# hilo-mpc/hilo-mpc

Measured on AMD Instinct MI355X. Metric: MPC steps/sec (batched instances, whole node) at fixed (nx,nu,N), higher is better.
Workload: dtype f64

## Files before the change

### hilo_mpc_amd/_lib.py

```python
import ctypes as C
import os

HERE = os.path.dirname(os.path.abspath(__file__))
LIB_PATH = os.environ.get('HILO_LIB_PATH') or os.path.join(HERE, 'libhilo_hip.so')

c_double_p = C.c_void_p
c_i64 = C.c_int64


class HiloError(RuntimeError):
    code = 0


class NotPositiveDefinite(HiloError, ValueError):
    code = -5


class KfDesc(C.Structure):
    _fields_ = [('model_id', C.c_int32), ('kind', C.c_int32), ('continuous', C.c_int32), ('erk_order', C.c_int32),
                ('n_sub', C.c_int32), ('lti_nx', C.c_int32), ('lti_nu', C.c_int32), ('lti_ny', C.c_int32),
                ('dt', C.c_double), ('alpha', C.c_double), ('beta', C.c_double), ('kappa', C.c_double),
                ('user_source', C.c_char_p), ('n_user_gp', C.c_int32), ('user_gp', C.c_void_p * 4)]


# ... 45 lines not shown
               [('user_source', C.c_char_p)] + \
               [(n, C.c_int32) for n in ('user_nx', 'user_nu', 'user_np', 'user_ny', 'user_discrete', 'collocation_degree')] + \
               [('coll_A', C.c_void_p), ('coll_D', C.c_void_p), ('n_con', C.c_int32), ('reserved6', C.c_int32), ('con_lb', C.c_void_p),
                ('con_ub', C.c_void_p)]


_lib = None


def _declare(lib):
    vp, i32, i64, dbl = C.c_void_p, C.c_int, C.c_int64, C.c_double
    P = C.POINTER
    sig = {
        'hilo_abi_version': (C.c_int, []),
        'hilo_last_error': (C.c_char_p, []),
        'hilo_device_count': (C.c_int, [P(C.c_int)]),
        'hilo_model_dims': (C.c_int, [i32, P(C.c_int), P(C.c_int), P(C.c_int), P(C.c_int), P(C.c_int)]),
        'hilo_malloc': (C.c_int, [P(vp), C.c_uint64, i32]),
        'hilo_free': (C.c_int, [vp]),
        'hilo_memcpy_h2d': (C.c_int, [vp, vp, C.c_uint64, vp]),
        'hilo_memcpy_d2h': (C.c_int, [vp, vp, C.c_uint64, vp]),
        'hilo_stream_sync': (C.c_int, [vp]),
        'hilo_kf_create': (C.c_int, [P(KfDesc), i32, P(vp)]),
        'hilo_kf_destroy': (None, [vp]),
        'hilo_kf_dims': (C.c_int, [vp, P(C.c_int), P(C.c_int), P(C.c_int), P(C.c_int), P(C.c_int)]),
        'hilo_kf_predict': (C.c_int, [vp, i64, vp, vp, i64, vp, i64, vp, vp]),
        'hilo_kf_update': (C.c_int, [vp, i64, vp, vp, vp, i64, vp, i64, vp, vp, vp]),
        'hilo_kf_step': (C.c_int, [vp, i64, vp, vp, vp, i64, vp, i64, vp, i64, vp, vp, vp]),
        'hilo_pf_function': (C.c_int, [vp, i64, i32, vp, vp, vp, i64, vp, vp, vp, i64, vp, vp, vp, vp]),
        'hilo_model_rollout': (C.c_int, [vp, P(SimOpts), i64, i32, vp, vp, i64, i64, vp, vp, vp, vp]),
        'hilo_model_rollout_resume': (C.c_int, [vp, P(SimOpts), i64, i32, vp, vp, i64, i64, vp, vp, vp, vp, vp]),
        'hilo_model_rollout_dae': (C.c_int, [vp, P(SimOpts), i64, i32, vp, vp, vp, i64, i64, vp, vp, vp, vp, vp]),
        'hilo_model_linearize': (C.c_int, [vp, i64, vp, vp, i64, vp, vp, vp, vp]),
        'hilo_lqr_gain': (C.c_int, [i32, i32, i64, vp, i64, vp, i64, vp, i64, vp, i64, vp, i64, P(LqrOpts), vp, vp, vp, vp]),
        'hilo_lqr_call': (C.c_int, [vp, P(LqrOpts), i64, vp, vp, vp, vp, i64, vp, vp, vp, vp, vp, vp, vp, vp]),
        'hilo_lqr_apply': (C.c_int, [i32, i32, i64, vp, i64, vp, vp, vp, vp, vp]),
        'hilo_pf_stats': (C.c_int, [vp, i64, i32, vp, vp, vp, vp, vp, vp, vp, vp, vp]),
        'hilo_pf_resample': (C.c_int, [vp, i64, i32, vp, vp, vp, vp, vp, vp, vp, vp]),
        'hilo_nmpc_create': (C.c_int, [P(NmpcDesc), i32, P(vp)]),
        'hilo_nmpc_destroy': (None, [vp]),
        'hilo_nmpc_dims': (C.c_int, [vp, P(C.c_int), P(C.c_int), P(C.c_int), P(C.c_int), P(C.c_int)]),
        'hilo_nmpc_reset_warm_start': (C.c_int, [vp]),
        'hilo_nmpc_set_fix_x0': (C.c_int, [vp, i32]),
        'hilo_nmpc_set_x0_box': (C.c_int, [vp, vp, vp]),
        'hilo_nmpc_set_gather': (C.c_int, [vp, vp, i32]),
        'hilo_nmpc_set_plant_out': (C.c_int, [vp, vp]),
        'hilo_nmpc_set_var_bounds': (C.c_int, [vp, vp, vp]),
        'hilo_kf_steps': (C.c_int, [vp, i64, i32, vp, vp, vp, i64, i64, vp, i64, vp, i64, vp, i32, vp, vp]),
        'hilo_kf_steps_split': (C.c_int, [vp, i64, i32, vp, vp, vp, i64, i64, vp, i64, vp, i64, vp, i64, vp, i32, vp, vp]),
        'hilo_nmpc_solve': (C.c_int, [vp, i64, vp, vp, i64, vp, vp, vp, vp, vp, vp, vp, vp, vp, vp]),
        'hilo_nmpc_solve_tv': (C.c_int, [vp, i64, vp, vp, i64, vp, vp, vp, vp, vp, vp, vp, vp, vp, vp]),
        'hilo_nmpc_profile': (C.c_int, [vp, i32, vp]),
        'hilo_nmpc_layout_capacity': (C.c_int, [i32, i32, P(C.c_int), P(C.c_longlong), P(C.c_longlong)]),
        'hilo_nmpc_plant_step': (C.c_int, [vp, i64, vp, vp, vp, i64, vp, vp]),
        'hilo_jit_precompile': (C.c_int, [C.c_char_p] + [i32] * 11),
        'hilo_nmpc_set_aux_outputs': (C.c_int, [vp, vp, vp]),
        'hilo_gp_set_mean_program': (C.c_int, [vp, vp, i32]),
        'hilo_jit_precompile_kf': (C.c_int, [C.c_char_p]),
        'hilo_mhe_create': (C.c_int, [P(MheDesc), i32, P(vp)]),
        'hilo_mhe_destroy': (None, [vp]),
        'hilo_mhe_dims': (C.c_int, [vp] + [P(C.c_int)] * 6),
        'hilo_mhe_reset_warm_start': (C.c_int, [vp]),
        'hilo_mhe_estimate': (C.c_int, [vp, i64, vp, vp, i64, vp, vp, vp, vp, vp, vp, vp, vp, vp, vp, vp]),
        'hilo_qp_create': (C.c_int, [i32, i32, i32, P(vp)]),
        'hilo_qp_destroy': (None, [vp]),
        'hilo_qp_set_options': (C.c_int, [vp, dbl, i32]),
        'hilo_qp_set_stages': (C.c_int, [vp, i32, i32, i32, P(i32)]),
        'hilo_qp_solve': (C.c_int, [vp, i64, vp, i64, vp, i64, vp, i64, vp, vp, i64, vp, vp, i64, vp, vp, vp, vp, vp, vp, vp]),
        'hilo_qp_solve_pinned': (C.c_int, [vp, i64, vp, i64, vp, i64, vp, i64, vp, vp, i64, vp, i32, i64, vp, vp, i64, vp, vp, vp, vp, vp,
                                           vp, vp]),
        'hilo_gp_create': (C.c_int, [i32, i32, i32, vp, vp, vp, i32, vp, i32, dbl, P(vp)]),
        'hilo_gp_destroy': (None, [vp]),
        'hilo_gp_log_marginal_likelihood': (C.c_int, [vp, P(C.c_double)]),
        'hilo_gp_refit': (C.c_int, [vp, vp, i32, dbl]),
        'hilo_gp_lml_gradient': (C.c_int, [vp, i32, vp, vp, vp, vp]),
        'hilo_gp_predict': (C.c_int, [vp, i64, vp, i32, vp, vp, vp]),
        'hilo_gp_kernel_matrix': (C.c_int, [i32, i32, vp, i32, i64, vp, i64, vp, vp, vp]),
        'hilo_gp_mean': (C.c_int, [i32, i32, vp, i32, i64, vp, vp, vp]),
        'hilo_ann_create': (C.c_int, [i32, i32, i32, i32, vp, vp, vp, vp, vp, vp, vp, vp, P(vp)]),
        'hilo_ann_destroy': (None, [vp]),
        'hilo_ann_predict': (C.c_int, [vp, i64, vp, i64, vp, i64, vp]),
    }
    for name, (res, args) in sig.items():
        if not hasattr(lib, name):
            continue
        fn = getattr(lib, name)
        fn.restype = res
        fn.argtypes = args
    return lib


def lib():
    global _lib
    if _lib is None:
        if not os.path.exists(LIB_PATH):
            raise HiloError(f"{LIB_PATH} not found: build it with `python -m hilo_mpc_amd._build` "
                            f"(hipcc --offload-arch=gfx950). hilo_mpc_amd has no CPU fallback.")
        try:
            _lib = _declare(C.CDLL(LIB_PATH))
        except OSError as e:
            raise HiloError(f"cannot load {LIB_PATH}: {e}") from e
    return _lib


COMPILED_ONLY = 1

# ... 12 lines not shown
```

### hilo_mpc_amd/csrc/hilo_nmpc.hip

```cpp
#include <stdlib.h>
#include <string.h>

#include "hilo_nmpc_gen.h"
#include "hilo_nmpc_track.h"

namespace hilo {

template <class M>
__global__ void plant_step_kernel(const OcpConst* __restrict__ pcg, int64_t batch, const double* __restrict__ x,
                                  const double* __restrict__ u, const double* __restrict__ par, int64_t par_stride,
                                  double* __restrict__ xn) {
  const int64_t b = (int64_t)blockIdx.x * blockDim.x + threadIdx.x;
  if (b >= batch) return;
  constexpr int NX = M::NX, NU = M::NU, NP = M::NP;
  double xv[NX], uv[NU > 0 ? NU : 1], pv[NP > 0 ? NP : 1], xo[NX];
#pragma unroll
  for (int i = 0; i < NX; ++i) xv[i] = x[b * NX + i];
#pragma unroll
  for (int i = 0; i < NU; ++i) uv[i] = u[b * NU + i];
#pragma unroll
  for (int i = 0; i < NP; ++i) pv[i] = par[b * par_stride + i];
  if constexpr (model_has_ext<M>::value) {
    const GpExt ext{pcg->ext, nullptr, 1, 0, 0, false};
    model_step<M>(pcg->order, pcg->nsub, xv, uv, pv, pcg->dt, xo, ext);
// ... 579 lines not shown

extern "C" int hilo_nmpc_solve(hilo_nmpc* h, int64_t batch, const double* x0, const double* p, int64_t p_stride,
                               const double* v0, const double* u_old, double* v_opt, double* f_opt, double* lam_g,
                               double* u0, int32_t* status, int32_t* iters, double* kkt, void* stream) {
  return nmpc_solve_impl(h, batch, x0, p, p_stride, nullptr, 0, v0, u_old, v_opt, f_opt, lam_g, u0, status, iters, kkt, stream);
}

extern "C" int hilo_nmpc_solve_tv(hilo_nmpc* h, int64_t batch, const double* x0, const double* stage_data, int64_t sd_stride,
                                  const double* v0, const double* u_old, double* v_opt, double* f_opt, double* lam_g,
                                  double* u0, int32_t* status, int32_t* iters, double* kkt, void* stream) {
  HILO_REQUIRE(h && (h->tv || h->tv_width), "hilo_nmpc_solve_tv: the handle was not created with desc.time_varying");
  HILO_REQUIRE(batch <= 0 || stage_data, "hilo_nmpc_solve_tv: NULL stage data");
  const int64_t need = (int64_t)(h->N + 1) * (h->nx + h->nu + h->np);
  HILO_REQUIRE(sd_stride == 0 || sd_stride >= need, "hilo_nmpc_solve_tv: sd_stride %lld < %lld", (long long)sd_stride,
               (long long)need);
  return nmpc_solve_impl(h, batch, x0, nullptr, 0, stage_data, sd_stride, v0, u_old, v_opt, f_opt, lam_g, u0, status, iters, kkt,
                         stream);
}

extern "C" int hilo_nmpc_profile(hilo_nmpc* h, int enable, long long* cycles_host) {
  HILO_REQUIRE(h, "hilo_nmpc_profile: NULL handle");
  HILO_HIP_CHECK(hipSetDevice(h->device));
  if (cycles_host && h->prof) {
    HILO_HIP_CHECK(hipDeviceSynchronize());
    HILO_HIP_CHECK(hipMemcpy(cycles_host, h->prof, sizeof(long long) * PH_COUNT, hipMemcpyDeviceToHost));
  }
  if (enable && !h->prof) {
    HILO_HIP_CHECK(hipMalloc((void**)&h->prof, sizeof(long long) * PH_COUNT));
    HILO_HIP_CHECK(hipMemset(h->prof, 0, sizeof(long long) * PH_COUNT));
  } else if (!enable && h->prof) {
    HILO_HIP_CHECK(hipFree(h->prof));
    h->prof = nullptr;
  }
  return HILO_OK;
}

extern "C" int hilo_nmpc_plant_step(hilo_nmpc* h, int64_t batch, const double* x, const double* u, const double* p,
                                    int64_t p_stride, double* x_next, void* stream) {
  HILO_REQUIRE(h, "hilo_nmpc_plant_step: NULL handle");
  if (batch <= 0) return HILO_OK;
  HILO_REQUIRE(x && u && x_next && (h->np == 0 || p), "hilo_nmpc_plant_step: NULL argument");
  HILO_HIP_CHECK(hipSetDevice(h->device));
  if (h->jit_policy >= 0) return jit_launch_plant(h->jit.plant, h->dev, batch, x, u, p, p_stride, x_next, (hipStream_t)stream);
  const unsigned grid = (unsigned)((batch + 255) / 256);
  switch (h->model_id) {
#define X(ID, T) case ID: hipLaunchKernelGGL((plant_step_kernel<T>), dim3(grid), dim3(256), 0, (hipStream_t)stream, h->dev, batch, x, u, p, p_stride, x_next); break;
    HILO_NMPC_MODELS(X)
#undef X
  }
  HILO_HIP_CHECK(hipGetLastError());
  return HILO_OK;
}

#ifdef HILO_OCP_DPROF
extern "C" int hilo_debug_dprof(long long* out, int reset) {
  if (out) HILO_HIP_CHECK(hipMemcpyFromSymbol(out, HIP_SYMBOL(hilo::g_dprof), sizeof(long long) * 32));
  if (reset) { long long z[32] = {0}; HILO_HIP_CHECK(hipMemcpyToSymbol(HIP_SYMBOL(hilo::g_dprof), z, sizeof(z))); }
  return HILO_OK;
}
#endif
```

### hilo_mpc_amd/csrc/hilo_ocp.h

```cpp
#pragma once
#include "hilo_colloc.h"
#include "hilo_common.h"
#include "hilo_models.h"

namespace hilo {

constexpr int OCP_MAXNX = 12, OCP_MAXNU = 8, OCP_MAXNZ = OCP_MAXNX + OCP_MAXNU;
constexpr int OCP_FILTER = 16;
constexpr int OCP_MAXNC = 16;
#ifndef HILO_OCP_TPB
#define HILO_OCP_TPB 64
#endif
#ifndef HILO_OCP_MINW
#define HILO_OCP_MINW 1
#endif
#ifdef HILO_OCP_INLINE_PHASES
#define OCP_PHASE __attribute__((always_inline))
#else
#define OCP_PHASE __attribute__((noinline))
#endif
#ifndef HILO_OCP_SEAMS
#define HILO_OCP_SEAMS 3
#endif
constexpr int OCP_SEAMS = HILO_OCP_SEAMS;
#ifndef HILO_OCP_LAYOUT_CAP
#define HILO_OCP_LAYOUT_CAP 1
#endif
constexpr bool OCP_LAYOUT_CAP = HILO_OCP_LAYOUT_CAP != 0;
constexpr int OCP_TPB = HILO_OCP_TPB;
constexpr int OCP_NCOST = 2 * OCP_MAXNZ * OCP_MAXNZ + 4 * OCP_MAXNZ + 64;

struct OcpConst {
  int N, order, nsub, max_iter, acceptable_iter, flags;
  int Nc;
  int tail_off;
  double dt;
  double lbz[OCP_MAXNZ], ubz[OCP_MAXNZ];
  double x0lb[OCP_MAXNX], x0ub[OCP_MAXNX];
  double sz[OCP_MAXNZ];
  double tol, acceptable_tol, mu_init, kappa_eps, kappa_mu, theta_mu, tau_min, bound_push, bound_frac, s_max,
      kappa_sigma, gamma_theta, gamma_phi, delta_ls, s_theta, s_phi, eta_phi, theta_min_fact, theta_max_fact,
      delta_w_min, delta_w_0, delta_w_max, kappa_w_minus, kappa_w_plus, kappa_w_plus_bar;
  const double* ext;
  unsigned x0_free_mask;
  unsigned k0_only_mask;
  int nc, nc_term;
  double dlb[OCP_MAXNC], dub[OCP_MAXNC];
  int n_con_ref, n_tcon_ref;
  short row_ref[OCP_MAXNC], trow_ref[OCP_MAXNC];
  CollData coll;
  unsigned long long pair_mask[4];
  double bound_relax;
  double cost[OCP_NCOST];
};

inline void ocp_default_options(OcpConst& c) {
  c.max_iter = 3000; c.acceptable_iter = 15;
  c.tol = 1e-8; c.acceptable_tol = 1e-6; c.mu_init = 0.1;
  c.kappa_eps = 10.0; c.kappa_mu = 0.2; c.theta_mu = 1.5; c.tau_min = 0.99;
  c.bound_push = 1e-2; c.bound_frac = 1e-2; c.s_max = 100.0; c.kappa_sigma = 1e10;
  c.gamma_theta = 1e-5; c.gamma_phi = 1e-8; c.delta_ls = 1.0; c.s_theta = 1.1; c.s_phi = 2.3; c.eta_phi = 1e-8;
  c.theta_min_fact = 1e-4; c.theta_max_fact = 1e4;
  c.delta_w_min = 1e-20; c.delta_w_0 = 1e-4; c.delta_w_max = 1e40; c.kappa_w_minus = 1.0 / 3; c.kappa_w_plus = 8.0;
  c.kappa_w_plus_bar = 100.0;
  for (auto& w : c.pair_mask) w = ~0ull;
}

struct OpSum { static constexpr bool NAN_VOTE = false; __device__ static double id() { return 0.0; } __device__ static double f(double a, double b) { return a + b; } };
__device__ __forceinline__ double nmax(double a, double b) { return (a != a || a > b) ? a : b; }
struct OpMax { static constexpr bool NAN_VOTE = true; __device__ static double id() { return -INFINITY; } __device__ static double f(double a, double b) { return nmax(a, b); } };
struct OpMin { static constexpr bool NAN_VOTE = false; __device__ static double id() { return INFINITY; } __device__ static double f(double a, double b) { return fmin(a, b); } };
struct OpMax2 { static constexpr bool NAN_VOTE = false; __device__ static double id() { return -INFINITY; } __device__ static double f(double a, double b) { return fmax(a, b); } };

template <int CTRL>
__device__ __forceinline__ double dpp_mov(double v) {
// ... 16 lines not shown
  return (int64_t)(((unsigned long long)hi << 32) | lo);
}
__device__ __forceinline__ double uni(double v) {
  return __hiloint2double(__builtin_amdgcn_readfirstlane(__double2hiint(v)), __builtin_amdgcn_readfirstlane(__double2loint(v)));
}
template <class T>
__device__ __forceinline__ __attribute__((address_space(3))) T* uni(__attribute__((address_space(3))) T* p) {
  return (__attribute__((address_space(3))) T*)(size_t)(unsigned)__builtin_amdgcn_readfirstlane((int)(size_t)p);
}
template <class T>
__device__ __forceinline__ T* uni(T* p) {
  const unsigned long long a = (unsigned long long)p;
  const unsigned lo = (unsigned)__builtin_amdgcn_readfirstlane((int)(unsigned)a);
  const unsigned hi = (unsigned)__builtin_amdgcn_readfirstlane((int)(unsigned)(a >> 32));
  return (T*)(((unsigned long long)hi << 32) | lo);
}
#ifndef HILO_RSQ_NEWTON
#define HILO_RSQ_NEWTON 2
#endif
__device__ __forceinline__ double rsq_fast(double x) {
  double y = __builtin_amdgcn_rsq(x);
  const double hx = 0.5 * x;
  y = y * fma(-hx * y, y, 1.5);
  if (HILO_RSQ_NEWTON >= 2) y = y * fma(-hx * y, y, 1.5);
  return y;
}
typedef double v4d __attribute__((ext_vector_type(4)));
struct FTheta { double f, theta, x; };

__device__ __forceinline__ bool wave_any_nan(double v) { return __builtin_amdgcn_ballot_w64(v != v) != 0ull; }
template <class Op>
__device__ __forceinline__ double wave_reduce(double v) {
  if constexpr (Op::NAN_VOTE) {
    const bool nan = wave_any_nan(v);
    const double r = wave_reduce<OpMax2>(v);
    return nan ? __builtin_nan("") : r;
  }
  v = Op::f(v, dpp_mov<0xB1>(v));
  v = Op::f(v, dpp_mov<0x4E>(v));
  v = Op::f(v, dpp_mov<0x141>(v));
  v = Op::f(v, dpp_mov<0x140>(v));
  return uni(Op::f(Op::f(read_lane(v, 0), read_lane(v, 16)), Op::f(read_lane(v, 32), read_lane(v, 48))));
}

enum { R_SUM = 0, R_MAX = 1, R_MIN = 2, R_MAX2 = 3 };
__device__ __forceinline__ double red_apply(int op, double a, double b) {
  switch (op) {
    case R_SUM: return a + b;
    case R_MAX: return fmax(a, b);
    case R_MIN: return fmin(a, b);
    default: return fmax(a, b);
  }
}
template <int... OPS>
struct WaveReduceN {
  static constexpr int n = sizeof...(OPS);
  template <int CTRL>
  __device__ __forceinline__ static void level(double* v) {
    constexpr int ops[n] = {OPS...};
    double t[n];
#pragma unroll
    for (int j = 0; j < n; ++j) t[j] = dpp_mov<CTRL>(v[j]);
#pragma unroll
    for (int j = 0; j < n; ++j) v[j] = red_apply(ops[j], v[j], t[j]);
  }
  __device__ __forceinline__ static void run(double* v) {
    static_assert(OCP_TPB == 64, "one wave per instance");
    constexpr int ops[n] = {OPS...};
    bool nan[n];
#pragma unroll
    for (int j = 0; j < n; ++j) nan[j] = ops[j] == R_MAX && wave_any_nan(v[j]);
    level<0xB1>(v);
    level<0x4E>(v);
    level<0x141>(v);
    level<0x140>(v);
    double a[n], b[n];
#pragma unroll
    for (int j = 0; j < n; ++j) {
      a[j] = red_apply(ops[j], read_lane(v[j], 0), read_lane(v[j], 16));
      b[j] = red_apply(ops[j], read_lane(v[j], 32), read_lane(v[j], 48));
    }
#pragma unroll
    for (int j = 0; j < n; ++j) {
      const double r = uni(red_apply(ops[j], a[j], b[j]));
      v[j] = nan[j] ? __builtin_nan("") : r;
    }
  }
};

template <class Op>
__device__ __forceinline__ double block_reduce(double v, __attribute__((address_space(3))) double* scratch) {
  v = wave_reduce<Op>(v);
  if constexpr (OCP_TPB == 64) return v;
  const int nw = blockDim.x >> 6;
  if (nw == 1) return v;
  __syncthreads();
  if ((threadIdx.x & 63) == 0) scratch[threadIdx.x >> 6] = v;
  __syncthreads();
  double r = Op::id();
  for (int w = 0; w < nw; ++w) r = Op::f(r, scratch[w]);
  return r;
}

template <class MS, class = void> struct sym_masks {
  static constexpr unsigned long long X = ~0ull, J = ~0ull, H = ~0ull;
};
template <class MS> struct sym_masks<MS, void_tt<decltype(MS::HAS_MASKS)>> {
  static constexpr unsigned long long X = MS::HAS_MASKS ? MS::XMASK : ~0ull, J = MS::HAS_MASKS ? MS::JMASK : ~0ull,
                                      H = MS::HAS_MASKS ? MS::HMASK : ~0ull;
};
template <class PB, class = void> struct pb_plant { static constexpr bool value = false; };
template <class PB> struct pb_plant<PB, void_tt<decltype(PB::PLANT)>> { static constexpr bool value = PB::PLANT; };
template <class PB, class = void> struct pb_symtab { static constexpr bool value = false; };
template <class PB> struct pb_symtab<PB, void_tt<decltype(PB::SYMTAB)>> { static constexpr bool value = PB::SYMTAB; };
template <class PB, class = void> struct pb_nh { static constexpr int value = 0; };
template <class PB> struct pb_nh<PB, void_tt<decltype(PB::NH)>> { static constexpr int value = PB::NH; };
template <class PB, class = void> struct pb_sym { static constexpr bool value = false; };
template <class PB> struct pb_sym<PB, void_tt<decltype(PB::SYM)>> { static constexpr bool value = PB::SYM; };
template <class PB, class = void> struct pb_sym_mhe { static constexpr bool value = false; };
template <class PB> struct pb_sym_mhe<PB, void_tt<decltype(PB::SYM_MHE)>> { static constexpr bool value = PB::SYM_MHE; };
template <class PB, class = void> struct pb_vec_n { static constexpr int value = 0; };
template <class PB> struct pb_vec_n<PB, void_tt<decltype(PB::VEC_N)>> { static constexpr int value = PB::VEC_N; };
template <class PB, class = void> struct pb_fused_con { static constexpr bool value = false; };
template <class PB> struct pb_fused_con<PB, void_tt<decltype(PB::FUSED_CON)>> { static constexpr bool value = PB::FUSED_CON; };
template <class PB, class = void> struct pb_prep { static constexpr int value = 0; };
template <class PB> struct pb_prep<PB, void_tt<decltype(PB::PREP)>> { static constexpr int value = PB::PREP; };
template <class PB, class = void> struct pb_vec_max { static constexpr int value = 3; };
template <class PB> struct pb_vec_max<PB, void_tt<decltype(PB::VEC_MAX)>> { static constexpr int value = PB::VEC_MAX; };
template <class PB, class = void> struct pb_cstage { static constexpr int value = 0; };
template <class PB> struct pb_cstage<PB, void_tt<decltype(PB::CSTAGE)>> { static constexpr int value = PB::CSTAGE; };
template <class PB, class = void> struct pb_xcw { static constexpr int value = 0; };
template <class PB> struct pb_xcw<PB, void_tt<decltype(PB::XCW)>> { static constexpr int value = PB::XCW; };
template <class PB, class = void> struct pb_lam_fix { static constexpr bool value = false; };
template <class PB> struct pb_lam_fix<PB, void_tt<decltype(PB::LAM_FIX)>> { static constexpr bool value = PB::LAM_FIX; };
template <class PB, class = void> struct pb_fused { static constexpr bool value = false; };
template <class PB> struct pb_fused<PB, void_tt<decltype(PB::FUSED)>> { static constexpr bool value = PB::FUSED; };
template <class PB, class = void> struct pb_layout_n { static constexpr int value = 0; };
template <class PB> struct pb_layout_n<PB, void_tt<decltype(PB::LAYOUT_N)>> { static constexpr int value = PB::LAYOUT_N; };

__host__ __device__ constexpr size_t ocp_iter_doubles(int NX, int NU, int NC, int N) {
  const size_t NZ = NX + NU, NDIR = NZ * (NZ + 1) / 2, S = (size_t)(N + 1) * NZ;
  return 9 * S + NX + 5 * (size_t)N * NX + (size_t)N * NX * (NZ + 1) + (size_t)N * NZ * (NZ + 1) + (size_t)(N + 1) * NDIR +
         (size_t)(N + 1) * NX * (NX + 1) + (size_t)N * NU * (NX + 1) + (size_t)N * NX * (NX + 1) + (size_t)N * NC * (14 + NZ) +
         (size_t)N * 4 * NX;
}
__host__ __device__ constexpr size_t ocp_fixed_doubles(int NX, int NU, int NCONST, int NPAR, int NSD, int NEXT, int N, int NPREP = 0) {
  const size_t NZ = NX + NU;
  return NCONST + NZ * NZ + NZ + (N + 1) + 2 * 16 + 16 + NPAR + (size_t)(N + 1) * (NSD > 0 ? NSD : 0) + 1 + NEXT +
         (NZ * (NZ + 1) / 2 + 2) / 2 + NPREP;
}

struct OcpExtra {
  const double* par2;
  int npar1;
// ... 1531 lines not shown
          lsum += ok[u] ? fabs(lv[u]) : 0.0;
        }
      }
    }
    double ncon = 0.0;
    if constexpr (NC > 0) {
      OCP_FOR(e, N * NC) {
        const int m = e % NC;
        double sg = 0.0, q = 0.0;
        if (row_on(pc, e / NC, m)) {
          dmax = nmax(dmax, fabs(-l.cnu[e] - l.cvL[e] + l.cvU[e]));
          pmax = nmax(pmax, fabs(l.cd[e] - l.cs[e]));
          th += fabs(l.cd[e] - l.cs[e]);
          lsum += fabs(l.cnu[e]);
          zsum += fabs(l.cvL[e]) + fabs(l.cvU[e]);
          if (pc.dlb[m] > -INFINITY) {
            const double sl = l.cs[e] - pc.dlb[m], is = rcp_fast(sl), p = sl * l.cvL[e];
            cmax = fmax(cmax, p);
            cmin = fmin(cmin, p);
            sg += l.cvL[e] * is;
            q += is;
          }
          if (pc.dub[m] < INFINITY) {
            const double su = pc.dub[m] - l.cs[e], is = rcp_fast(su), p = su * l.cvU[e];
            cmax = fmax(cmax, p);
            cmin = fmin(cmin, p);
            sg += l.cvU[e] * is;
            q -= is;
          }
        }
        l.csig[e] = sg;
        l.crb[e] = q;
      }
      ncon = (double)N * pc.nc + pc.nc_term;
    }
    KktErr r;
    DTICK(12)
    if constexpr (OCP_TPB == 64) {
      double rv[7] = {th, cmax, cmin, dmax, pmax, lsum, zsum};
      WaveReduceN<R_SUM, R_MAX2, R_MIN, R_MAX, R_MAX, R_SUM, R_SUM>::run(rv);
      r.theta = rv[0]; r.pmax = rv[1]; r.pmin = rv[2]; dmax = rv[3]; pmax = rv[4]; lsum = rv[5]; zsum = rv[6];
    } else {
      r.theta = uni(block_reduce<OpSum>(th, l.red));
      r.pmax = uni(block_reduce<OpMax2>(cmax, l.red));
      r.pmin = uni(block_reduce<OpMin>(cmin, l.red));
      dmax = block_reduce<OpMax>(dmax, l.red);
      pmax = block_reduce<OpMax>(pmax, l.red);
      lsum = block_reduce<OpSum>(lsum, l.red);
      zsum = block_reduce<OpSum>(zsum, l.red);
    }
    const double i_smax = rcp_fast(pc.s_max);
    const double s_d = fmax(pc.s_max, (lsum + zsum) * rcp_fast(N * NX + ncon + nb)) * i_smax;
    const double poison = (lsum + zsum + r.theta) * 0.0;
    r.s_c = uni(fmax(pc.s_max, zsum * rcp_fast(nb)) * i_smax + poison);
    r.i_s_c = uni(rcp_fast(r.s_c));
    r.dual_s = uni(dmax * rcp_fast(s_d));
    r.prim = uni(pmax);
    DTICK(13)
    return r;
  }
  __device__ __forceinline__ static double compl_of(const KktErr& r, double mu) { return fmax(fmax(r.pmax - mu, mu - r.pmin), 0.0); }
  __device__ __forceinline__ static bool switching(const OcpConst& pc, double alpha, double nd, double th0) {
    const double dls = pc.delta_ls;
    const bool plain = alpha > 1e-30 && alpha < 1e30 && nd > 1e-100 && nd < 1e100 && th0 > 1e-100 && th0 < 1e100 && dls > 1e-30 && dls < 1e30;
    if (plain) {
      auto lg2 = [](double x) {
        return (double)__builtin_amdgcn_frexp_exp(x) + (double)__builtin_amdgcn_logf((float)__builtin_amdgcn_frexp_mant(x));
      };
      const double d = lg2(alpha) + pc.s_phi * lg2(nd) - lg2(dls) - pc.s_theta * lg2(th0);
      if (fabs(d) > 1e-4) return d > 0.0;
    }
    return alpha * pow(nd, pc.s_phi) > dls * pow(th0, pc.s_theta);
  }
  __device__ static void finish_rhs(const Lds l, double mu) {
    const OcpConst& pc = *(const OcpConst*)l.pc;
    const int N = pc.N;
    {
      constexpr int U = BIG ? 3 : 2;
      const int SLT = (N + 1) * NZ;
      for (int base = 0; base < SLT; base += OCP_TPB * U) {
        double gr[U], qv[U];
        bool ok[U];
#pragma unroll
        for (int u = 0; u < U; ++u) {
          const int e0 = base + u * OCP_TPB + (int)threadIdx.x;
          ok[u] = e0 < SLT;
          const int e = ok[u] ? e0 : 0, k = e / NZ, i = e - k * NZ;
          gr[u] = l.grad[e];
          qv[u] = k < N ? l.W[(size_t)(k * NZ + i) * WP + NZ] : l.rbN[i < NX ? i : 0];
        }
#pragma unroll
        for (int u = 0; u < U; ++u) {
          const int e = base + u * OCP_TPB + (int)threadIdx.x;
          if (!ok[u]) continue;
          const int k = e / NZ, i = e - k * NZ;
          if (k < N) l.W[(size_t)(k * NZ + i) * WP + NZ] = gr[u] - mu * qv[u];
          else if (i < NX) l.rbN[i] = gr[u] - mu * qv[u];
        }
      }
    }
    if constexpr (NC > 0) {
      OCP_FOR(e, N * NC) l.crb[e] = -mu * l.crb[e];
    }
    __syncthreads();
  }
  __device__ static double count_bounds(const Lds l) {
    const OcpConst& pc = *(const OcpConst*)l.pc;
    const int N = pc.N;
    double nb = 0.0;
// ... 980 lines not shown
      if constexpr (NC > 0) {
        OCP_FOR(e, N * NC) {
          const int m = e % NC;
          double sg = 0.0, r = 0.0;
          if (row_on(pc, e / NC, m)) {
            if (pc.dlb[m] > -INFINITY) { const double is = 1.0 / (l.cs[e] - pc.dlb[m]); sg += mu_r * is * is; r -= mu_r * is; }
            if (pc.dub[m] < INFINITY) { const double is = 1.0 / (pc.dub[m] - l.cs[e]); sg += mu_r * is * is; r += mu_r * is; }
          }
          l.csig[e] = sg;
          l.crb[e] = r;
        }
      }
      __syncthreads();
      riccati(lbase, ws, mu, 1.0, true);
      double a = 1.0, dmax = 0.0;
      if constexpr (NC > 0) {
        OCP_FOR(e, N * NC) {
          const int m = e % NC;
          if (!row_on(pc, e / NC, m)) continue;
          const double d = l.cds[e];
          if (pc.dlb[m] > -INFINITY && d < 0.0) a = fmin(a, -tau * (l.cs[e] - pc.dlb[m]) / d);
          if (pc.dub[m] < INFINITY && d > 0.0) a = fmin(a, tau * (pc.dub[m] - l.cs[e]) / d);
        }
      }
      OCP_FOR(e, SL) {
        const double d = l.D[e], lb = l.lbA[e], ub = l.ubA[e], z = l.Z[e];
        dmax = nmax(dmax, fabs(d));
        if (lb > -INFINITY && d < 0.0) a = fmin(a, -tau * (z - lb) / d);
        if (ub < INFINITY && d > 0.0) a = fmin(a, tau * (ub - z) / d);
      }
      double alpha = block_reduce<OpMin>(a, l.red);
      dmax = block_reduce<OpMax>(dmax, l.red);
      if (dmax <= 1e-9 && th > 1e-6) return 2;
      bool ok = false;
      double tht = 0.0, ft = 0.0;
      while (alpha > 1e-10) {
        OCP_FOR(e, SL) l.Zt[e] = l.Z[e] + alpha * l.D[e];
        if constexpr (NC > 0)
          OCP_FOR(e, N * NC) l.cst[e] = l.cs[e] + alpha * l.cds[e];
        __syncthreads();
        const FTheta trial = eval_values(lbase, ws, l.Zt, l.ct, l.cst);
        ft = trial.f; tht = trial.theta;
        if (isfinite(tht) && tht <= (1.0 - 1e-4 * alpha) * th) { ok = true; break; }
        alpha = uni(alpha * 0.5);
      }
      if (!ok) return th > 1e-6 ? 2 : 1;
      OCP_FOR(e, SL) l.Z[e] = l.Zt[e];
      if constexpr (NC > 0)
        OCP_FOR(e, N * NC) l.cs[e] = l.cst[e];
      __syncthreads();
      th = tht;
      if (th <= 0.9 * th_start && th <= theta_max) {
        const double ph = ft + mu * barrier_logs(l, l.Z, l.cs);
        bool acc = true;
        for (int q = 0; q < nfilt; ++q)
          if (th >= l.filt[2 * q] && ph >= l.filt[2 * q + 1]) { acc = false; break; }
        if (acc) return 0;
      }
      eval_derivs(lbase, ws);
    }
    return 1;
  }
  __device__ OCP_PHASE static void load_instance(lds_double* lds_raw_in, double* ws_in, const OcpConst* pcg_in, int64_t b_in,
                                                 const double* x0_in, const double* par_in, int64_t par_stride_in,
                                                 const double* sdata_in, int64_t sd_stride_in, const double* vb_in, int v_prefix_in,
                                                 const double* par2_in, int npar1_in, const double* lbx_in, const double* ubx_in,
                                                 int64_t bx_stride_in) {
    using S = Ocp<PB>;
    constexpr int NTAIL = NX - NXV - NH;
    using gbl_const = const __attribute__((address_space(1))) OcpConst;
    lds_double* const lds_raw = uni(lds_raw_in);
    double* const wsb = uni(ws_in);
    gbl_const* const pcg = (gbl_const*)uni(pcg_in);
    const int64_t b = uni(b_in), par_stride = uni(par_stride_in), sd_stride = uni(sd_stride_in), bx_stride = uni(bx_stride_in);
    gbl_cdouble *const x0 = (gbl_cdouble*)uni(x0_in), *const par = (gbl_cdouble*)uni(par_in), *const sdata = (gbl_cdouble*)uni(sdata_in),
                *const vb = (gbl_cdouble*)uni(vb_in), *const par2 = (gbl_cdouble*)uni(par2_in), *const lbx = (gbl_cdouble*)uni(lbx_in),
                *const ubx = (gbl_cdouble*)uni(ubx_in);
    const int v_prefix = uni(v_prefix_in), npar1 = uni(npar1_in);
    const int t = threadIdx.x;
    const int N = uni(pcg->N);
    const Lds l = carve(lds_raw, wsb, N);
    constexpr int CT = (S::NCONST + OCP_TPB - 1) / OCP_TPB, PT = (PB::NPAR + OCP_TPB - 1) / OCP_TPB;
    gbl_cdouble* const csrc = reinterpret_cast<gbl_cdouble*>(pcg);
    double cbuf[CT], pbuf[PT > 0 ? PT : 1];
#pragma unroll
    for (int j = 0; j < CT; ++j) {
      const int i = j * OCP_TPB + t;
      cbuf[j] = csrc[i < S::NCONST ? i : 0];
    }
    {
      const int n1 = par2 || npar1 > 0 ? npar1 : PB::NPAR;
      const bool has1 = n1 > 0, has2 = par2 != nullptr && n1 < PB::NPAR;
#pragma unroll
      for (int j = 0; j < PT; ++j) {
        const int i = j * OCP_TPB + t;
        const bool p1 = i < PB::NPAR && i < n1, p2 = i < PB::NPAR && !p1 && has2;
        double v1 = 0.0, v2 = 0.0;
        if (has1) v1 = par[b * par_stride + (p1 ? i : 0)];
        if (has2) v2 = par2[b * (int64_t)(PB::NPAR - n1) + (p2 ? i - n1 : 0)];
        pbuf[j] = p1 ? v1 : (p2 ? v2 : 0.0);
      }
    }
    const int SL = (N + 1) * NZ;
    const int flags_g = uni(pcg->flags), tail_g = uni(pcg->tail_off), Ncv = NH > 0 ? uni(pcg->Nc) : N;
    FreeTest is_free_g;
    is_free_g.pinm = uni((int)(FIX_X0 ? (~pcg->x0_free_mask) & ((1u << NX) - 1u) : 0u));
    is_free_g.N = N;
    is_free_g.Nc = NH > 0 ? Ncv : 0;
    const int toff = tail_g > 0 ? tail_g : (N + 1) * NXV + Ncv * NU;
    struct SlotIn { double raw, lo, up; bool pin, bx; };
// ... 276 lines not shown
    if constexpr (NC > 0) {
      OCP_FOR(e, N * NC) {
        const int m = e % NC;
        double dl = 0.0, du = 0.0;
        if (S::row_on(pc, e / NC, m)) {
          const double d = l.cds[e];
          if (pc.dlb[m] > -INFINITY) {
            const double is = rcp_fast(l.cs[e] - pc.dlb[m]), vl = l.cvL[e];
            dl = mu * is - vl - vl * is * d;
            r_p = fmax(r_p, -d * is);
            r_z = fmax(r_z, -dl * rcp_fast(vl));
          }
          if (pc.dub[m] < INFINITY) {
            const double is = rcp_fast(pc.dub[m] - l.cs[e]), vu = l.cvU[e];
            du = mu * is - vu + vu * is * d;
            r_p = fmax(r_p, d * is);
            r_z = fmax(r_z, -du * rcp_fast(vu));
          }
          dphi += l.crb[e] * d;
        }
        l.cdvL[e] = dl;
        l.cdvU[e] = du;
      }
    }
    DTICK(15)
    if constexpr (OCP_TPB == 64) {
      double rv[3] = {r_p, r_z, dphi};
      WaveReduceN<R_MAX, R_MAX, R_SUM>::run(rv);
      r_p = rv[0]; r_z = rv[1]; dphi = rv[2];
    } else {
      r_p = block_reduce<OpMax>(r_p, l.red);
      r_z = block_reduce<OpMax>(r_z, l.red);
      dphi = block_reduce<OpSum>(dphi, l.red);
    }
    const double a_p = uni(r_p > tau ? tau / r_p : 1.0), a_z = uni(r_z > tau ? tau / r_z : 1.0);
    if (!blog_ok) blog = S::barrier_logs(l, l.Z, l.cs);
    const double phi0 = uni(fval + mu * blog);
    DTICK(16)
    OCP_TICK(PH_STEP)
    double alpha = a_p;
    bool accepted = false, armijo = false;
    double blog_t = 0.0, f_acc = 0.0;
    for (int ls = 0; ls < 60; ++ls) {
      DTICKR
      const double blog_part = S::form_trial_part(l, alpha);
      DTICK(17)
      tprof[PH_NLS] += 1;
      const FTheta trial = S::eval_values(lds_raw, wsb, l.Zt, l.ct, l.cst, l.cdt, blog_part);
      blog_t = trial.x;
      DTICK(18)
      const double ft = trial.f, tht = trial.theta;
      const double pht = uni(ft + mu * blog_t);
      bool ok = isfinite(pht) && isfinite(tht) && tht <= theta_max;
      if (ok) {
        for (int q = 0; q < nfilt; ++q) {
          const double tf = l.filt[2 * q], pf = l.filt[2 * q + 1];
          if (tht >= tf && pht - 10 * 2.220446049250313e-16 * fabs(pf) >= pf) { ok = false; break; }
        }
      }
      bool sw = false;
      if (ok) {
        sw = th0 <= theta_min && dphi < 0.0 && S::switching(pc, alpha, -dphi, th0);
        const double rnd = 10 * 2.220446049250313e-16 * fabs(phi0);
        if (sw) ok = pht - phi0 - rnd <= pc.eta_phi * alpha * dphi;
        else ok = tht <= (1 - pc.gamma_theta) * th0 || pht - phi0 - rnd <= -pc.gamma_phi * th0;
      }
      DTICK(19)
      if (ok) { accepted = true; armijo = sw; f_acc = ft; break; }
      if (ls == 0 && tht >= th0) {
        OCP_FOR(e, N * NX) l.c0[e] = l.c[e];
        if constexpr (NC > 0)
          OCP_FOR(e, N * NC) l.cd0[e] = l.cd[e];
        double a_prev = alpha, th_old = tht;
        bool soc_ok = false, soc_sw = false;
        for (int ps = 0; ps < 4; ++ps) {
          OCP_FOR(e, N * NX) l.c[e] = a_prev * l.c[e] + l.ct[e];
          if constexpr (NC > 0) {
            OCP_FOR(e, N * NC) {
              if (S::row_on(pc, e / NC, e % NC)) l.cd[e] = l.cs[e] + a_prev * (l.cd[e] - l.cs[e]) + (l.cdt[e] - l.cst[e]);
            }
          }
          __syncthreads();
          tprof[PH_NRIC] += 1;
          if (!uni(S::riccati(lds_raw, wsb, mu, delta))) break;
          double a = 1.0;
          OCP_FOR(e, SL) {
            const double d = l.D[e], lb = l.lbA[e], ub = l.ubA[e], z = l.Z[e];
            if (lb > -INFINITY && d < 0.0) a = fmin(a, -tau * (z - lb) / d);
            if (ub < INFINITY && d > 0.0) a = fmin(a, tau * (ub - z) / d);
          }
          if constexpr (NC > 0) {
            OCP_FOR(e, N * NC) {
              const int m = e % NC;
              if (!S::row_on(pc, e / NC, m)) continue;
              const double d = l.cds[e];
              if (pc.dlb[m] > -INFINITY && d < 0.0) a = fmin(a, -tau * (l.cs[e] - pc.dlb[m]) / d);
              if (pc.dub[m] < INFINITY && d > 0.0) a = fmin(a, tau * (pc.dub[m] - l.cs[e]) / d);
            }
          }
          const double a_s = block_reduce<OpMin>(a, l.red);
          const double blog_part2 = S::form_trial_part(l, a_s);
          tprof[PH_NLS] += 1;
          const FTheta t2 = S::eval_values(lds_raw, wsb, l.Zt, l.ct, l.cst, l.cdt, blog_part2);
          blog_t = t2.x;
          const double ths = t2.theta;
          const double phs = uni(t2.f + mu * blog_t);
          bool oks = isfinite(phs) && isfinite(ths) && ths <= theta_max;
          if (oks) {
            for (int q = 0; q < nfilt; ++q) {
              const double tf = l.filt[2 * q], pf = l.filt[2 * q + 1];
              if (ths >= tf && phs - 10 * 2.220446049250313e-16 * fabs(pf) >= pf) { oks = false; break; }
            }
          }
          if (oks) {
            const bool sw2 = th0 <= theta_min && dphi < 0.0 && S::switching(pc, alpha, -dphi, th0);
            const double rnd = 10 * 2.220446049250313e-16 * fabs(phi0);
            if (sw2) oks = phs - phi0 - rnd <= pc.eta_phi * alpha * dphi;
            else oks = ths <= (1 - pc.gamma_theta) * th0 || phs - phi0 - rnd <= -pc.gamma_phi * th0;
            if (oks) { soc_ok = true; soc_sw = sw2; f_acc = t2.f; break; }
          }
          if (!(ths <= 0.99 * th_old)) break;
          th_old = ths;
          a_prev = a_s;
        }
        if (soc_ok) {
          OCP_FOR(e, N * NX) {
            const double cs0 = l.c0[e];
            l.c0[e] = l.lamn[e];
            l.c[e] = cs0;
          }
          if constexpr (NC > 0) {
            OCP_FOR(e, N * NC) {
              const double cd0 = l.cd0[e];
              l.cd0[e] = l.cnun[e];
              l.cd[e] = cd0;
            }
          }
          __syncthreads();
          tprof[PH_NRIC] += 1;
          (void)uni(S::riccati(lds_raw, wsb, mu, delta));
          OCP_FOR(e, N * NX) l.lamn[e] = l.c0[e];
          if constexpr (NC > 0)
            OCP_FOR(e, N * NC) l.cnun[e] = l.cd0[e];
          __syncthreads();
          accepted = true; armijo = soc_sw; break;
        }
        OCP_FOR(e, N * NX) l.c[e] = l.c0[e];
        if constexpr (NC > 0)
          OCP_FOR(e, N * NC) l.cd[e] = l.cd0[e];
        __syncthreads();
        tprof[PH_NRIC] += 1;
        (void)uni(S::riccati(lds_raw, wsb, mu, delta));
      }
      alpha = uni(alpha * 0.5);
      double amin = pc.gamma_theta;
      if (dphi < 0.0) {
        amin = fmin(amin, pc.gamma_phi * th0 / (-dphi));
        if (th0 <= theta_min) amin = fmin(amin, pc.delta_ls * pow(th0, pc.s_theta) / pow(-dphi, pc.s_phi));
      }
      if (alpha < 0.05 * amin) break;
    }
    OCP_TICK(PH_LS)
    DTICKR
    const bool do_resto = !accepted;
    if (!armijo || do_resto) {
      if (nfilt == OCP_FILTER) {
// ... 241 lines not shown
```

### include/hilo_hip.h

```cpp
#ifndef HILO_HIP_H
#define HILO_HIP_H

#include <stdint.h>

#ifdef __cplusplus
extern "C" {
#endif

#define HILO_ABI_VERSION 1

#define HILO_OK 0
#define HILO_EINVAL (-1)
#define HILO_ENOMEM (-2)
#define HILO_EHIP (-3)
#define HILO_ENOTSUP (-4)
#define HILO_COMPILED_ONLY 1
#define HILO_ENOTPD (-5)

#define HILO_MODEL_LTI 0
#define HILO_MODEL_TOY1D 1
#define HILO_MODEL_BIOREACTOR3 2
#define HILO_MODEL_CHEMOSTAT4 3
#define HILO_MODEL_PENDULUM4 4
#define HILO_MODEL_ROBOT6 5
// ... 239 lines not shown
  int32_t acc_soft;
  const double* acc_max_violation;
} hilo_nmpc_desc;

#define HILO_MODEL_USER 100
int hilo_jit_precompile(const char* user_source, int policy, int nth, int ne, int nc, int coll_d, int N, int hold, int cont,
                        int tv, int big, int has_fun);

#define HILO_X_CONST 0
#define HILO_X_VARX 1
#define HILO_X_VARU 2
#define HILO_X_VARP 3
#define HILO_X_ADD 10
#define HILO_X_SUB 11
#define HILO_X_MUL 12
#define HILO_X_DIV 13
#define HILO_X_NEG 14
#define HILO_X_SQ 15
#define HILO_X_SIN 16
#define HILO_X_COS 17
#define HILO_X_EXP 18
#define HILO_X_LOG 19
#define HILO_X_SQRT 20
#define HILO_X_POWI 21

int hilo_nmpc_create(const hilo_nmpc_desc* desc, int device, hilo_nmpc** out);
void hilo_nmpc_destroy(hilo_nmpc* h);
int hilo_nmpc_dims(const hilo_nmpc* h, int* n_v, int* n_g, int* nx, int* nu, int* np);
int hilo_nmpc_reset_warm_start(hilo_nmpc* h);
int hilo_nmpc_set_aux_outputs(hilo_nmpc* h, double* g, double* lam_x);
int hilo_nmpc_set_gather(hilo_nmpc* h, double* table, int stride);
int hilo_nmpc_set_plant_out(hilo_nmpc* h, double* x_next);
int hilo_nmpc_set_var_bounds(hilo_nmpc* h, const double* lbx, const double* ubx);
int hilo_nmpc_set_fix_x0(hilo_nmpc* h, int fix_x0);
int hilo_nmpc_set_x0_box(hilo_nmpc* h, const double* x0_lb_host, const double* x0_ub_host);
int hilo_nmpc_solve(hilo_nmpc* h, int64_t batch,
                    const double* x0,
                    const double* p, int64_t p_stride,
                    const double* v0,
                    const double* u_old,
                    double* v_opt,
                    double* f_opt,
                    double* lam_g,
                    double* u0,
                    int32_t* status,
                    int32_t* iters,
                    double* kkt,
                    void* stream);
int hilo_nmpc_solve_tv(hilo_nmpc* h, int64_t batch, const double* x0, const double* stage_data, int64_t sd_stride,
                       const double* v0, const double* u_old, double* v_opt, double* f_opt, double* lam_g, double* u0,
                       int32_t* status, int32_t* iters, double* kkt, void* stream);
int hilo_nmpc_profile(hilo_nmpc* h, int enable, long long* cycles_host);
int hilo_nmpc_layout_capacity(int model_id, int taylor, int* n_cap, long long* lds_cap, long long* lds_next);
int hilo_nmpc_plant_step(hilo_nmpc* h, int64_t batch, const double* x, const double* u, const double* p,
                         int64_t p_stride, double* x_next, void* stream);

typedef struct hilo_mhe hilo_mhe;

typedef struct hilo_mhe_desc {
  int32_t model_id, N, erk_order, n_sub, max_iter, acceptable_iter;
  double dt, tol, acceptable_tol, mu_init, bound_relax_factor;
  const double* Wx;
  const double* Wy;
  const double* Ww;
  const double* x_lb; const double* x_ub; const double* w_lb; const double* w_ub;
  const double* x_scaling; const double* w_scaling; const double* u_scaling;
  const double* x_guess; const double* w_guess;
  int32_t estimate_parameters;
  int32_t reserved;
  const double* Wp;
  const double* p_lb; const double* p_ub; const double* p_scaling; const double* p_guess;
  const char* user_source;
  int32_t user_nx, user_nu, user_np, user_ny, user_discrete, collocation_degree;
  const double* coll_A;
  const double* coll_D;
  int32_t n_con; int32_t reserved6;
  const double* con_lb; const double* con_ub;
} hilo_mhe_desc;

int hilo_mhe_create(const hilo_mhe_desc* desc, int device, hilo_mhe** out);
void hilo_mhe_destroy(hilo_mhe* h);
int hilo_mhe_dims(const hilo_mhe* h, int* n_v, int* n_g, int* nx, int* nu, int* np, int* ny);
int hilo_mhe_reset_warm_start(hilo_mhe* h);
int hilo_mhe_estimate(hilo_mhe* h, int64_t batch,
                      const double* x_arrival,
                      const double* p, int64_t p_stride,
                      const double* u_meas,
                      const double* y_meas,
                      const double* v0,
                      double* v_opt, double* f_opt, double* lam_g,
                      double* x_opt,
                      int32_t* status, int32_t* iters, double* kkt, void* stream);

typedef struct hilo_qp hilo_qp;
int hilo_qp_create(int n, int m, int device, hilo_qp** out);
void hilo_qp_destroy(hilo_qp* h);
int hilo_qp_set_options(hilo_qp* h, double tol , int max_iter );
int hilo_qp_set_stages(hilo_qp* h, int nx, int nu, int N, int* used);
int hilo_qp_solve(hilo_qp* h, int64_t batch,
                  const double* H, int64_t h_stride,
                  const double* g, int64_t g_stride,
                  const double* A, int64_t a_stride,
                  const double* lbx, const double* ubx, int64_t bx_stride,
                  const double* lba, const double* uba, int64_t ba_stride,
                  double* x,
                  double* f,
// ... 31 lines not shown
```

Before: 7.399 million.

## Use transposed multi-value wave reductions and ballot-based filter checks in OCP solver

Adds a transposed wave reduction that packs up to four same-type reductions into one DPP/permlane butterfly, so several sums or maxes share the cross-lane steps instead of each value being reduced separately. Filter-dominance checks in the line search are replaced by a per-lane compare plus a wave ballot instead of a serial loop over filter entries. Both are enabled by default through a new seams bitmask value. A self-test entry point compares the new reduction against the old one. The new reduction adds lane-select and permlane-swap overhead and relies on permlane16/32 swap instructions. The ballot check assumes the filter has no more than 64 entries.

```diff
diff --git a/hilo_mpc_amd/_lib.py b/hilo_mpc_amd/_lib.py
--- a/hilo_mpc_amd/_lib.py
+++ b/hilo_mpc_amd/_lib.py
@@ -121,6 +121,7 @@
         'hilo_nmpc_solve_tv': (C.c_int, [vp, i64, vp, vp, i64, vp, vp, vp, vp, vp, vp, vp, vp, vp, vp]),
         'hilo_nmpc_profile': (C.c_int, [vp, i32, vp]),
         'hilo_nmpc_layout_capacity': (C.c_int, [i32, i32, P(C.c_int), P(C.c_longlong), P(C.c_longlong)]),
+        'hilo_ocp_reduce_selftest': (C.c_int, [i32, P(C.c_int), vp, vp, vp, vp]),
         'hilo_nmpc_plant_step': (C.c_int, [vp, i64, vp, vp, vp, i64, vp, vp]),
         'hilo_jit_precompile': (C.c_int, [C.c_char_p] + [i32] * 11),
         'hilo_nmpc_set_aux_outputs': (C.c_int, [vp, vp, vp]),
diff --git a/hilo_mpc_amd/csrc/hilo_nmpc.hip b/hilo_mpc_amd/csrc/hilo_nmpc.hip
--- a/hilo_mpc_amd/csrc/hilo_nmpc.hip
+++ b/hilo_mpc_amd/csrc/hilo_nmpc.hip
@@ -655,6 +655,42 @@
   return HILO_OK;
 }
 
+template <int... OPS>
+__global__ void __launch_bounds__(64) reduce_selftest_kernel(const double* in, double* out_new, double* out_plain) {
+  constexpr int n = sizeof...(OPS);
+  double a[n], b[n];
+  for (int j = 0; j < n; ++j) a[j] = b[j] = in[threadIdx.x * n + j];
+  WaveReduceN<OPS...>::run_transposed(a);
+  WaveReduceN<OPS...>::run_plain(b);
+  if (threadIdx.x == 0)
+    for (int j = 0; j < n; ++j) { out_new[j] = a[j]; out_plain[j] = b[j]; }
+}
+template <int... OPS>
+static bool reduce_selftest_try(int n, const int* ops, const double* in, double* out_new, double* out_plain, hipStream_t s) {
+  constexpr int want[] = {OPS...};
+  if (n != (int)sizeof...(OPS)) return false;
+  for (int j = 0; j < n; ++j)
+    if (ops[j] != want[j]) return false;
+  hipLaunchKernelGGL((reduce_selftest_kernel<OPS...>), dim3(1), dim3(64), 0, s, in, out_new, out_plain);
+  return true;
+}
+extern "C" int hilo_ocp_reduce_selftest(int n, const int* ops, const double* in, double* out_new, double* out_plain, void* stream) {
+  HILO_REQUIRE(n >= 1 && n <= 8 && ops && in && out_new && out_plain, "hilo_ocp_reduce_selftest: bad argument");
+  hipStream_t s = (hipStream_t)stream;
+  constexpr int S = R_SUM, M = R_MAX, I = R_MIN, P = R_MAX2;
+#define T(...) reduce_selftest_try<__VA_ARGS__>(n, ops, in, out_new, out_plain, s)
+  const bool ok = T(S) || T(M) || T(I) || T(P) ||
+                  T(S, S) || T(M, M) || T(I, M) || T(S, P) ||
+                  T(S, S, S) || T(M, M, S) || T(I, S, P) ||
+                  T(S, S, S, S) || T(P, I, M, M) || T(S, M, I, P) ||
+                  T(S, P, I, M, M, S, S) || T(S, S, S, S, S, S, S) ||
+                  T(S, S, S, S, S, S, S, S) || T(S, P, I, M, M, S, S, M) || T(M, P, M, I, P, M, I, M);
+#undef T
+  if (!ok) return fail(HILO_EINVAL, "hilo_ocp_reduce_selftest: this mix of %d operations is not compiled in", n);
+  HILO_HIP_CHECK(hipGetLastError());
+  return HILO_OK;
+}
+
 #ifdef HILO_OCP_DPROF
 extern "C" int hilo_debug_dprof(long long* out, int reset) {
   if (out) HILO_HIP_CHECK(hipMemcpyFromSymbol(out, HIP_SYMBOL(hilo::g_dprof), sizeof(long long) * 32));
diff --git a/hilo_mpc_amd/csrc/hilo_ocp.h b/hilo_mpc_amd/csrc/hilo_ocp.h
--- a/hilo_mpc_amd/csrc/hilo_ocp.h
+++ b/hilo_mpc_amd/csrc/hilo_ocp.h
@@ -20,7 +20,7 @@
 #define OCP_PHASE __attribute__((noinline))
 #endif
 #ifndef HILO_OCP_SEAMS
-#define HILO_OCP_SEAMS 3
+#define HILO_OCP_SEAMS 15
 #endif
 constexpr int OCP_SEAMS = HILO_OCP_SEAMS;
 #ifndef HILO_OCP_LAYOUT_CAP
@@ -143,6 +143,7 @@
     default: return fmax(a, b);
   }
 }
+typedef unsigned ocp_u2 __attribute__((ext_vector_type(2)));
 template <int... OPS>
 struct WaveReduceN {
   static constexpr int n = sizeof...(OPS);
@@ -155,7 +156,7 @@
 #pragma unroll
     for (int j = 0; j < n; ++j) v[j] = red_apply(ops[j], v[j], t[j]);
   }
-  __device__ __forceinline__ static void run(double* v) {
+  __device__ __forceinline__ static void run_plain(double* v) {
     static_assert(OCP_TPB == 64, "one wave per instance");
     constexpr int ops[n] = {OPS...};
     bool nan[n];
@@ -176,6 +177,85 @@
       const double r = uni(red_apply(ops[j], a[j], b[j]));
       v[j] = nan[j] ? __builtin_nan("") : r;
     }
+  }
+  template <bool SUM>
+  __device__ __forceinline__ static double gop(double a, double b) { return SUM ? a + b : fmax(a, b); }
+  template <bool SUM, int CTRL>
+  __device__ __forceinline__ static double link(double keep, double send) { return gop<SUM>(keep, dpp_mov<CTRL>(send)); }
+  template <bool SUM, bool ROW32>
+  __device__ __forceinline__ static double row_link(double w) {
+    const unsigned lo = (unsigned)__double2loint(w), hi = (unsigned)__double2hiint(w);
+    const ocp_u2 a = ROW32 ? __builtin_amdgcn_permlane32_swap(lo, lo, false, false) : __builtin_amdgcn_permlane16_swap(lo, lo, false, false);
+    const ocp_u2 b = ROW32 ? __builtin_amdgcn_permlane32_swap(hi, hi, false, false) : __builtin_amdgcn_permlane16_swap(hi, hi, false, false);
+    return gop<SUM>(__hiloint2double((int)b.x, (int)a.x), __hiloint2double((int)b.y, (int)a.y));
+  }
+  template <bool SUM, int C>
+  __device__ __forceinline__ static void group(double* g, bool b0, bool b1) {
+    static_assert(C >= 1 && C <= 4, "groups of up to four values");
+    double w;
+    if constexpr (C == 1) {
+      w = link<SUM, 0xB1>(g[0], g[0]);
+      w = link<SUM, 0x4E>(w, w);
+    } else if constexpr (C == 2) {
+      w = link<SUM, 0xB1>(b0 ? g[1] : g[0], b0 ? g[0] : g[1]);
+      w = link<SUM, 0x4E>(w, w);
+    } else {
+      const double w0 = link<SUM, 0xB1>(b0 ? g[2] : g[0], b0 ? g[0] : g[2]);
+      const double w1 = C == 4 ? link<SUM, 0xB1>(b0 ? g[3] : g[1], b0 ? g[1] : g[3]) : link<SUM, 0xB1>(g[1], g[1]);
+      w = link<SUM, 0x4E>(b1 ? w1 : w0, b1 ? w0 : w1);
+    }
+    w = link<SUM, 0x141>(w, w);
+    w = link<SUM, 0x140>(w, w);
+    w = row_link<SUM, false>(w);
+    w = row_link<SUM, true>(w);
+    if constexpr (C <= 2) {
+#pragma unroll
+      for (int k = 0; k < C; ++k) g[k] = read_lane(w, k);
+    } else {
+#pragma unroll
+      for (int k = 0; k < C; ++k) g[k] = read_lane(w, (k >> 1) | ((k & 1) << 1));
+    }
+  }
+  template <bool SUM>
+  __device__ __forceinline__ static void groups(double* v, bool b0, bool b1) {
+    constexpr int ops[n] = {OPS...};
+    int idx[n] = {};
+    int c = 0;
+#pragma unroll
+    for (int j = 0; j < n; ++j)
+      if ((ops[j] == R_SUM) == SUM) idx[c++] = j;
+#pragma unroll
+    for (int base = 0; base < n; base += 4) {
+      double g[4];
+#pragma unroll
+      for (int k = 0; k < 4; ++k)
+        if (base + k < c) g[k] = ops[idx[base + k]] == R_MIN ? -v[idx[base + k]] : v[idx[base + k]];
+      const int left = c - base;
+      if (left >= 4) group<SUM, 4>(g, b0, b1);
+      else if (left == 3) group<SUM, 3>(g, b0, b1);
+      else if (left == 2) group<SUM, 2>(g, b0, b1);
+      else if (left == 1) group<SUM, 1>(g, b0, b1);
+#pragma unroll
+      for (int k = 0; k < 4; ++k)
+        if (base + k < c) v[idx[base + k]] = ops[idx[base + k]] == R_MIN ? -g[k] : g[k];
+    }
+  }
+  __device__ __forceinline__ static void run_transposed(double* v) {
+    static_assert(OCP_TPB == 64, "one wave per instance");
+    constexpr int ops[n] = {OPS...};
+    bool nan[n];
+#pragma unroll
+    for (int j = 0; j < n; ++j) nan[j] = ops[j] == R_MAX && wave_any_nan(v[j]);
+    const unsigned t = threadIdx.x;
+    const bool b0 = ((t ^ (t >> 2)) & 1u) != 0, b1 = ((t ^ (t >> 1)) & 2u) != 0;
+    groups<true>(v, b0, b1);
+    groups<false>(v, b0, b1);
+#pragma unroll
+    for (int j = 0; j < n; ++j) v[j] = nan[j] ? __builtin_nan("") : v[j];
+  }
+  __device__ __forceinline__ static void run(double* v) {
+    if constexpr (OCP_SEAMS & 4) run_transposed(v);
+    else run_plain(v);
   }
 };
 
@@ -191,6 +271,23 @@
   double r = Op::id();
   for (int w = 0; w < nw; ++w) r = Op::f(r, scratch[w]);
   return r;
+}
+
+template <bool MARGIN>
+__device__ __forceinline__ bool filter_dominates(const lds_double* filt, int nfilt, double th, double ph) {
+  if constexpr (OCP_TPB == 64 && (OCP_SEAMS & 8)) {
+    if (nfilt == 0) return false;
+    const int q = (int)threadIdx.x < nfilt ? (int)threadIdx.x : 0;
+    const double tf = filt[2 * q], pf = filt[2 * q + 1];
+    const bool hit = MARGIN ? (th >= tf && ph - 10 * 2.220446049250313e-16 * fabs(pf) >= pf) : (th >= tf && ph >= pf);
+    return __builtin_amdgcn_ballot_w64(hit) != 0ull;
+  } else {
+    for (int q = 0; q < nfilt; ++q) {
+      const double tf = filt[2 * q], pf = filt[2 * q + 1];
+      if (MARGIN ? (th >= tf && ph - 10 * 2.220446049250313e-16 * fabs(pf) >= pf) : (th >= tf && ph >= pf)) return true;
+    }
+    return false;
+  }
 }
 
 template <class MS, class = void> struct sym_masks {
@@ -1828,9 +1925,11 @@
     const double i_smax = rcp_fast(pc.s_max);
     const double s_d = fmax(pc.s_max, (lsum + zsum) * rcp_fast(N * NX + ncon + nb)) * i_smax;
     const double poison = (lsum + zsum + r.theta) * 0.0;
-    r.s_c = uni(fmax(pc.s_max, zsum * rcp_fast(nb)) * i_smax + poison);
-    r.i_s_c = uni(rcp_fast(r.s_c));
-    r.dual_s = uni(dmax * rcp_fast(s_d));
+    const double s_c = fmax(pc.s_max, zsum * rcp_fast(nb)) * i_smax + poison;
+    const double i_s_c = rcp_fast(s_c), i_s_d = rcp_fast(s_d);
+    r.s_c = uni(s_c);
+    r.i_s_c = uni(i_s_c);
+    r.dual_s = uni(dmax * i_s_d);
     r.prim = uni(pmax);
     DTICK(13)
     return r;
@@ -2917,10 +3016,7 @@
       th = tht;
       if (th <= 0.9 * th_start && th <= theta_max) {
         const double ph = ft + mu * barrier_logs(l, l.Z, l.cs);
-        bool acc = true;
-        for (int q = 0; q < nfilt; ++q)
-          if (th >= l.filt[2 * q] && ph >= l.filt[2 * q + 1]) { acc = false; break; }
-        if (acc) return 0;
+        if (!filter_dominates<false>(l.filt, nfilt, th, ph)) return 0;
       }
       eval_derivs(lbase, ws);
     }
@@ -3303,12 +3399,7 @@
       const double ft = trial.f, tht = trial.theta;
       const double pht = uni(ft + mu * blog_t);
       bool ok = isfinite(pht) && isfinite(tht) && tht <= theta_max;
-      if (ok) {
-        for (int q = 0; q < nfilt; ++q) {
-          const double tf = l.filt[2 * q], pf = l.filt[2 * q + 1];
-          if (tht >= tf && pht - 10 * 2.220446049250313e-16 * fabs(pf) >= pf) { ok = false; break; }
-        }
-      }
+      if (ok) ok = !filter_dominates<true>(l.filt, nfilt, tht, pht);
       bool sw = false;
       if (ok) {
         sw = th0 <= theta_min && dphi < 0.0 && S::switching(pc, alpha, -dphi, th0);
@@ -3357,12 +3448,7 @@
           const double ths = t2.theta;
           const double phs = uni(t2.f + mu * blog_t);
           bool oks = isfinite(phs) && isfinite(ths) && ths <= theta_max;
-          if (oks) {
-            for (int q = 0; q < nfilt; ++q) {
-              const double tf = l.filt[2 * q], pf = l.filt[2 * q + 1];
-              if (ths >= tf && phs - 10 * 2.220446049250313e-16 * fabs(pf) >= pf) { oks = false; break; }
-            }
-          }
+          if (oks) oks = !filter_dominates<true>(l.filt, nfilt, ths, phs);
           if (oks) {
             const bool sw2 = th0 <= theta_min && dphi < 0.0 && S::switching(pc, alpha, -dphi, th0);
             const double rnd = 10 * 2.220446049250313e-16 * fabs(phi0);
diff --git a/include/hilo_hip.h b/include/hilo_hip.h
--- a/include/hilo_hip.h
+++ b/include/hilo_hip.h
@@ -315,6 +315,7 @@
                        int32_t* status, int32_t* iters, double* kkt, void* stream);
 int hilo_nmpc_profile(hilo_nmpc* h, int enable, long long* cycles_host);
 int hilo_nmpc_layout_capacity(int model_id, int taylor, int* n_cap, long long* lds_cap, long long* lds_next);
+int hilo_ocp_reduce_selftest(int n, const int* ops, const double* in, double* out_new, double* out_plain, void* stream);
 int hilo_nmpc_plant_step(hilo_nmpc* h, int64_t batch, const double* x, const double* u, const double* p,
                          int64_t p_stride, double* x_next, void* stream);
 
```

Result: faster. 7.481 million (median of 6 runs) (+1.1%).
